# SrikarK-code/clip-dplm

Measured on AMD Instinct MI355X. Metric: seq-pairs/sec/node, contrastive training step, ESM-2-35M dual encoder, higher is better.
Workload: dtype bf16

## Files before the change

### clip_dplm_amd/_ffi.py

```python
from __future__ import annotations

import ctypes as C
import os

_HERE = os.path.dirname(os.path.abspath(__file__))
LIB_PATH = os.path.join(_HERE, "lib", "libclipk.so")

BF16, F32, U8 = 0, 1, 2
SAME_CLASS = {"mask": 0, "positive": 1}
ACT_NONE, ACT_RELU, ACT_GELU, ACT_CELU, ACT_SOFTPLUS = 0, 1, 2, 3, 4
ACT = {None: ACT_NONE, "none": ACT_NONE, "relu": ACT_RELU, "gelu": ACT_GELU, "celu": ACT_CELU, "softplus": ACT_SOFTPLUS}


class ClipkError(RuntimeError):
    pass


class GemmArgs(C.Structure):
    _fields_ = [
        ("A", C.c_void_p), ("lda", C.c_int64),
        ("B", C.c_void_p), ("ldb", C.c_int64),
        ("C", C.c_void_p), ("ldc", C.c_int64), ("c_dtype", C.c_int),
        ("M", C.c_int), ("N", C.c_int), ("K", C.c_int),
        ("bias", C.c_void_p),
        ("act", C.c_int),
        ("out_preact", C.c_void_p), ("ldp", C.c_int64),
        ("dact_aux", C.c_void_p), ("ldd", C.c_int64),
        ("dact", C.c_int),
        ("residual", C.c_void_p), ("ldr", C.c_int64), ("r_dtype", C.c_int),
        ("alpha", C.c_float),
        ("drop_p", C.c_float), ("drop_seed", C.c_uint32),
        ("rope_cos", C.c_void_p), ("rope_sin", C.c_void_p),
        ("rope_L", C.c_int), ("rope_hd", C.c_int), ("rope_cols", C.c_int), ("rope_row0", C.c_int),
        ("aux_dtype", C.c_int),
        ("rope_interleaved", C.c_int),
    ]


_vp, _i, _i64, _f, _sz = C.c_void_p, C.c_int, C.c_int64, C.c_float, C.c_size_t

SIGNATURES = {
    "clipk_version": (_i, []),
    "clipk_arch": (C.c_char_p, []),
    "clipk_status_string": (C.c_char_p, [_i]),
    "clipk_set_option": (_i, [C.c_char_p, _i]),
    "clipk_get_option": (_i, [C.c_char_p, C.POINTER(_i)]),
    "clipk_reset_options": (_i, []),
    "clipk_gemm_nt": (_i, [C.POINTER(GemmArgs), _vp]),
    "clipk_gemm_wgrad_workspace": (_sz, [_i, _i, _i]),
    "clipk_gemm_wgrad": (_i, [_vp, _i64, _vp, _i64, _vp, _i64, _vp, _i, _i, _i, _i, _i, _i, _vp, _sz, _vp]),
    "clipk_simce_workspace": (_sz, [_i, _i, _i]),
    "clipk_simce_lse": (_i, [_vp, _i, _vp, _i, _vp, _i, _i, _vp, _i, _vp, _vp, _vp, _sz, _vp]),
    "clipk_simce_grad": (_i, [_vp, _i, _vp, _i, _vp, _i, _i, _vp, _i, _vp, _vp, _f, _f, _f, _vp, _vp, _vp, _sz, _vp]),
    "clipk_simce_grad_scaled": (_i, [_vp, _i, _vp, _i, _vp, _i, _i, _vp, _i, _vp, _vp, _f, _f, _f, _vp, _vp, _vp, _vp, _sz, _vp]),
    "clipk_ce_combine": (_i, [_vp, _vp, _vp, _vp, _i, _f, _f, _f, _vp, _vp]),
    "clipk_simce_cls_workspace": (_sz, [_i, _i, _i]),
    "clipk_simce_lse_cls": (_i, [_vp, _i, _vp, _i, _vp, _i, _i, _vp, _i, _vp, _vp, _i, _f, _vp, _vp, _vp, _vp, _sz, _vp]),
    "clipk_simce_grad_cls": (_i, [_vp, _i, _vp, _i, _vp, _i, _i, _vp, _i, _vp, _vp, _vp, _vp, _vp, _vp, _i, _f, _i, _f, _f,
                                  _f, _vp, _vp, _vp, _vp, _sz, _vp]),
    "clipk_simce_hard_workspace": (_sz, [_i, _i, _i]),
    "clipk_simce_lse_hard": (_i, [_vp, _i, _vp, _i, _vp, _i, _i, _vp, _f, _i, _vp, _vp, _vp, _vp, _vp, _vp, _sz, _vp]),
    "clipk_simce_grad_hard": (_i, [_vp, _i, _vp, _i, _vp, _i, _i, _vp, _f, _i, _vp, _vp, _vp, _vp, _f, _f, _f, _vp, _vp,
                                   _vp, _vp, _sz, _vp]),
    "clipk_simce_pairs_workspace": (_sz, [_i, _i, _i]),
    "clipk_simce_lse_pairs": (_i, [_vp, _i, _i, _i, C.POINTER(_i), _i, _vp, _vp, _vp, _vp, _sz, _vp]),
# ... 99 lines not shown

def load() -> C.CDLL:
    global _lib
    if _lib is not None:
        return _lib
    if not os.path.exists(LIB_PATH):
        raise ClipkError(
            f"{LIB_PATH} not found: the HIP extension is mandatory (there is no CPU fallback). "
            "Build it with `make` or `python -c 'import __graft_entry__ as g; g.build()'`.")
    lib = C.CDLL(LIB_PATH)
    lib.clipk_version.restype = C.c_int
    got = lib.clipk_version()
    if got != ABI_VERSION:
        raise ClipkError(f"{LIB_PATH} has ABI version {got}, this binding expects {ABI_VERSION}: rebuild it (`make`)")
    for name, (res, args) in SIGNATURES.items():
        fn = getattr(lib, name)
        fn.restype = res
        fn.argtypes = args
    _lib = lib
    return lib


def check(status: int, what: str) -> None:
    if status != 0:
        msg = load().clipk_status_string(status).decode()
        raise ClipkError(f"{what} failed: {msg} (status {status})")


def ptr(t):
    return None if t is None else t.data_ptr()

# ... 5 lines not shown
```

### clip_dplm_amd/csrc/gemm_wgrad.hip

```cpp
#include "common.h"
#include <stdlib.h>

struct clipk_wgrad_v3_args {
  const unsigned short* dY; long lddy;
  const unsigned short* X; long ldx;
  float* slab; float* bslab;
  int M, N, K;
  int ntn, ntk, splits, m_per_split;
};
extern "C" void clipk_wgrad_v3_plan(int M, int N, int K, int* ntn, int* ntk, int* splits, int* mps);
extern "C" int clipk_wgrad_v3_launch(const clipk_wgrad_v3_args* a, void* stream);

namespace {

constexpr int BN = 128, BKO = 128, BMS = 64, NTHREADS = 256;
constexpr int ROWB = 256;
constexpr int TILE_BYTES = BMS * ROWB;
constexpr int LDS_BYTES = 2 * TILE_BYTES;

struct WP {
  const unsigned short* dY; long lddy;
  const unsigned short* X; long ldx;
  float* slab;
  float* bslab;
  int M, N, K;
  int ntn, ntk, splits, m_per_split;
// ... 245 lines not shown
  p.dY = (const unsigned short*)dY; p.lddy = lddy;
  p.X = (const unsigned short*)X; p.ldx = ldx;
  p.slab = (float*)workspace;
  p.bslab = dbias ? (float*)workspace + (size_t)pl.splits * N * K : nullptr;
  p.M = M; p.N = N; p.K = K;
  p.ntn = pl.ntn; p.ntk = pl.ntk; p.splits = pl.splits; p.m_per_split = pl.mps;
  hipLaunchKernelGGL(wgrad_kernel, dim3(pl.ntn * pl.ntk * pl.splits), dim3(NTHREADS), LDS_BYTES, st, p);
  int rc = clipk_check_launch();
  if (rc) return rc;
  long total4 = (long)N * K / 4;
  int blocks = (int)((total4 + 255) / 256); if (blocks > 2048) blocks = 2048; if (blocks < 1) blocks = 1;
  hipLaunchKernelGGL(wgrad_reduce_kernel, dim3(blocks), dim3(256), 0, st, (const float*)p.slab, (const float*)p.bslab,
                     pl.splits, pl.splits, N, K, dW, (long)lddw, dbias, accumulate, il_hd, il_rows);
  return clipk_check_launch();
}
```

### clip_dplm_amd/csrc/gemm_wgrad_v3.hip

```cpp
#include "common.h"
#include <stdlib.h>
#include <type_traits>

struct clipk_wgrad_v3_args {
  const unsigned short* dY; long lddy;
  const unsigned short* X; long ldx;
  float* slab;
  float* bslab;
  int M, N, K;
  int ntn, ntk, splits, m_per_split;
};

namespace {

constexpr int BN = 256, BKO = 256, BMS = 64;
constexpr int ROWB = 256;
constexpr int HALF_BYTES = BMS * ROWB;
constexpr int BUF_BYTES = 4 * HALF_BYTES;
constexpr int LDS_BYTES = 2 * BUF_BYTES;
constexpr int YH0 = 0, YH1 = HALF_BYTES, XH0 = 2 * HALF_BYTES, XH1 = 3 * HALF_BYTES;

typedef __attribute__((ext_vector_type(2))) unsigned int u32x2;

template <int OFF>
// ... 13 lines not shown
template <int KH, int NH>
__device__ __forceinline__ void quad(f32x4 (&acc)[8][4], const bf16x8 (&yf)[4][2], const bf16x8 (&xf)[2][2][2]) {
#pragma unroll
  for (int ms = 0; ms < 2; ++ms)
#pragma unroll
    for (int u = 0; u < 2; ++u)
#pragma unroll
      for (int t = 0; t < 4; ++t)
        acc[NH * 4 + t][KH * 2 + u] =
            __builtin_amdgcn_mfma_f32_16x16x32_bf16(yf[t][ms], xf[KH][u][ms], acc[NH * 4 + t][KH * 2 + u], 0, 0, 0);
}

#define CLIPK_SB() __builtin_amdgcn_sched_barrier(0)
#define CLIPK_BAR() __builtin_amdgcn_s_barrier()

template <int SCHED>
__global__ __launch_bounds__(512, 1) void wgrad_v3_kernel(const clipk_wgrad_v3_args p) {
  extern __shared__ __attribute__((aligned(16))) char smem[];
  const int tid = threadIdx.x, lane = tid & 63;
  const int wid = __builtin_amdgcn_readfirstlane(tid >> 6);
  const int wn = wid >> 2, wk = wid & 3;
  const int ntiles = p.ntn * p.ntk;
  const int bid = xcd_remap(blockIdx.x, gridDim.x);
  const int split = bid / ntiles;
  const int tile = bid - split * ntiles;
  const int tn = tile / p.ntk, tk = tile - tn * p.ntk;
  const int n0 = tn * BN, k0 = tk * BKO;
  const int M = p.M, N = p.N, K = p.K;
  const int m_beg = split * p.m_per_split;
  int m_end = m_beg + p.m_per_split; m_end = m_end < M ? m_end : M;
  const int nkt = (m_end - m_beg + BMS - 1) / BMS;
  const bool has_bias = p.bslab != nullptr;
  int bias_T = tk;

  unsigned yv[2], xv[2];
#pragma unroll
  for (int i = 0; i < 2; ++i) {
    const int row = 4 * (2 * wid + i) + (lane >> 4);
    const int slot = lane & 15;
    const int col = (((slot >> 1) ^ (row & 7)) << 4) + (slot & 1) * 8;
    yv[i] = (unsigned)(((long)row * p.lddy + (col >> 6) * 128 + (col & 63)) * 2);
    xv[i] = (unsigned)(((long)row * p.ldx + (col >> 5) * 64 + (col & 31)) * 2);
  }
  const unsigned short* y_end = p.dY + ((long)(M - 1) * p.lddy + N);
  const unsigned short* x_end = p.X + ((long)(M - 1) * p.ldx + K);
  auto stage = [&](bool is_y, int half, int T, int region) {
    const long mt = (long)m_beg + (long)T * BMS;
    const unsigned short* base = is_y ? p.dY + mt * p.lddy + (n0 + half * 64) : p.X + mt * p.ldx + (k0 + half * 32);
// ... 5 lines not shown
    for (int i = 0; i < 2; ++i)
      __builtin_amdgcn_raw_ptr_buffer_load_lds(d, (__attribute__((address_space(3))) void*)(dst + i * 1024), 16,
                                               (int)(is_y ? yv[i] : xv[i]), 0, 0, 0);
  };
  auto stage1 = [&](bool is_y, int half, int T, int region, int i) {
    const long mt = (long)m_beg + (long)T * BMS;
    const unsigned short* base = is_y ? p.dY + mt * p.lddy + (n0 + half * 64) : p.X + mt * p.ldx + (k0 + half * 32);
    const long left = ((is_y ? y_end : x_end) - base) * 2;
    const int bytes = left > 0 ? (int)(left < 0x7fffffffL ? left : 0x7fffffffL) : 0;
    const auto d = __builtin_amdgcn_make_buffer_rsrc((void*)base, 0, bytes, 0x00020000);
    char* dst = smem + (T & 1) * BUF_BYTES + region + wid * 2048 + i * 1024;
    __builtin_amdgcn_raw_ptr_buffer_load_lds(d, (__attribute__((address_space(3))) void*)dst, 16,
                                             (int)(is_y ? (i ? yv[1] : yv[0]) : (i ? xv[1] : xv[0])), 0, 0, 0);
  };

  f32x4 acc[8][4];
#pragma unroll
  for (int i = 0; i < 8; ++i)
#pragma unroll
    for (int j = 0; j < 4; ++j) acc[i][j] = f32x4{0.f, 0.f, 0.f, 0.f};
  f32x4 accb[2][2];
#pragma unroll
  for (int u = 0; u < 2; ++u) { accb[u][0] = f32x4{0.f, 0.f, 0.f, 0.f}; accb[u][1] = accb[u][0]; }
  bf16x8 ones;
#pragma unroll
  for (int j = 0; j < 8; ++j) ones[j] = (short)0x3F80;

  const int g = lane >> 4, li = lane & 15;
  const int trow = 4 * g + (li >> 2);
  const int sw = trow & 7;
  const unsigned lds0 = (unsigned)(size_t)(__attribute__((address_space(3))) char*)smem;
  unsigned ya[4], xa[2];
#pragma unroll
  for (int t = 0; t < 4; ++t) ya[t] = lds0 + trow * ROWB + (((wn * 4 + t) ^ sw) << 5) + 8 * (li & 3);
#pragma unroll
  for (int u = 0; u < 2; ++u) xa[u] = lds0 + trow * ROWB + (((wk * 2 + u) ^ sw) << 5) + 8 * (li & 3);

  if constexpr (SCHED == 1) {
// ... 219 lines not shown

    stage(true, 0, 0, YH0); stage(false, 0, 0, XH0); stage(false, 1, 0, XH1); stage(true, 1, 0, YH1);
    if (nkt > 1) {
      stage(true, 0, 1, YH0); stage(false, 0, 1, XH0); stage(false, 1, 1, XH1); stage(true, 1, 1, YH1);
      asm volatile("s_waitcnt vmcnt(8)" ::: "memory");
    } else {
      asm volatile("s_waitcnt vmcnt(0)" ::: "memory");
    }
    CLIPK_SB(); CLIPK_BAR(); CLIPK_SB();
    read_yq(I0{}, 0u); read_x(I0{}, 0u);
    for (int T = 0; T < nkt - 2; ++T) step2(std::integral_constant<int, 0>{}, T);
    if (nkt > 1) step2(std::integral_constant<int, 1>{}, nkt - 2);
    step2(std::integral_constant<int, 2>{}, nkt - 1);
  }

  float* slab = p.slab + (long)split * N * K;
#pragma unroll
  for (int i = 0; i < 8; ++i)
#pragma unroll
    for (int r = 0; r < 4; ++r) {
      const int n = n0 + wn * 128 + i * 16 + 4 * g + r;
#pragma unroll
      for (int j = 0; j < 4; ++j) {
        const int k = k0 + wk * 64 + j * 16 + li;
        if (n < N && k < K) slab[(long)n * K + k] = acc[i][j][r];
      }
    }
  if (has_bias && li == 0) {
    float* bs = p.bslab + ((long)split * p.ntk + tk) * N;
#pragma unroll
    for (int u = 0; u < 2; ++u)
#pragma unroll
      for (int r = 0; r < 4; ++r) {
        const int n = n0 + wn * 128 + u * 64 + wk * 16 + 4 * g + r;
        if (n < N) bs[n] = accb[u][0][r] + accb[u][1][r];
      }
  }
}

}

extern "C" void clipk_wgrad_v3_plan(int M, int N, int K, int* ntn, int* ntk, int* splits, int* mps) {
  *ntn = (N + BN - 1) / BN; *ntk = (K + BKO - 1) / BKO;
  const int ntiles = *ntn * *ntk;
  int s = 256 / ntiles;
  if (clipk_opt_get(OPT_WGRAD_SPLITS) > 0) s = clipk_opt_get(OPT_WGRAD_SPLITS);
  if (s < 1) s = 1;
  const int max_splits = (M + 8 * BMS - 1) / (8 * BMS);
  if (s > max_splits) s = max_splits;
  int m = (M + s - 1) / s;
  m = (m + BMS - 1) / BMS * BMS;
// ... 4 lines not shown
extern "C" int clipk_wgrad_v3_launch(const clipk_wgrad_v3_args* a, void* stream) {
  static std::atomic<uint64_t> attr_set{0};
  clipk_once_per_device(attr_set, [&] {
    (void)hipFuncSetAttribute(reinterpret_cast<const void*>(wgrad_v3_kernel<1>),
                              hipFuncAttributeMaxDynamicSharedMemorySize, LDS_BYTES);
    (void)hipFuncSetAttribute(reinterpret_cast<const void*>(wgrad_v3_kernel<2>),
                              hipFuncAttributeMaxDynamicSharedMemorySize, LDS_BYTES);
  });
  const dim3 grid(a->ntn * a->ntk * a->splits);
  if (clipk_opt_get(OPT_WGRAD_KERNEL) == 3)
    hipLaunchKernelGGL(wgrad_v3_kernel<1>, grid, dim3(512), LDS_BYTES, (hipStream_t)stream, *a);
  else
    hipLaunchKernelGGL(wgrad_v3_kernel<2>, grid, dim3(512), LDS_BYTES, (hipStream_t)stream, *a);
  return clipk_check_launch();
}
```

### clip_dplm_amd/encoders.py

```python
from __future__ import annotations

import math
from typing import List, Optional

import os

import torch
import torch.nn as nn

from . import functional as KF
from . import ops


def _rope_tables(L: int, hd: int, device, theta: float = 10000.0):
    inv = 1.0 / (theta ** (torch.arange(0, hd, 2, dtype=torch.float32) / hd))
    fr = torch.arange(L, dtype=torch.float32)[:, None] * inv[None, :]
    return fr.cos().contiguous().to(device), fr.sin().contiguous().to(device)


WGRAD_SIDE_STREAM = False
_SIDE = {}


PREROTATE_QK = os.environ.get("CLIPK_PREROTATE", "1") != "0"
ROPE_IN_QKV_EPILOGUE = os.environ.get("CLIPK_ROPE_EPILOGUE", "1") != "0"
DIRECT_PARAM_GRADS = True
ROPE_INTERLEAVED = os.environ.get("CLIPK_ROPE_INTERLEAVED", "1") != "0"


def _direct_ok(t):
    g = t.grad if (t is not None and t.is_leaf) else None
    return g is not None and g.dtype == torch.float32 and g.is_contiguous() and g.device == t.device


def _fused_views(parts):
    p0 = parts[0]
    if not all(q.is_leaf and q.requires_grad and q.grad is not None and q.is_contiguous() and q.grad.is_contiguous()
               and q.dtype == torch.float32 and q.grad.dtype == torch.float32 for q in parts):
        return None
    d_ptr, g_ptr = p0.data_ptr(), p0.grad.data_ptr()
    for q in parts:
# ... 14 lines not shown

def _ln_bwd(dy, x, w, b, mean, rstd, pool=None, **kw):
    if pool is not None:
        wrow, B, L = pool
        if DIRECT_PARAM_GRADS and _direct_ok(w) and _direct_ok(b):
            dx, dxb, _, _ = ops.layernorm_meanpool_bwd(dy, wrow, x, w, mean, rstd, B, L, dgamma=w.grad, dbeta=b.grad,
                                                       accumulate=True, **kw)
            return dx, dxb, None, None
        return ops.layernorm_meanpool_bwd(dy, wrow, x, w, mean, rstd, B, L, **kw)
    if DIRECT_PARAM_GRADS and _direct_ok(w) and _direct_ok(b):
        dx, dxb, _, _ = ops.layernorm_bwd(dy, x, w, None, mean, rstd, dgamma=w.grad, dbeta=b.grad, accumulate=True, **kw)
        return dx, dxb, None, None
    return ops.layernorm_bwd(dy, x, w, None, mean, rstd, **kw)


def _wgrad(dy, x, lin=None, il=(0, 0)):
    if DIRECT_PARAM_GRADS and lin is not None and lin.gw is not None and lin.gb is not None:
        direct, kw = True, dict(dw=lin.gw, dbias=lin.gb, accumulate=True)
    else:
        direct = DIRECT_PARAM_GRADS and lin is not None and _direct_ok(lin.w) and _direct_ok(lin.b)
        kw = dict(dw=lin.w.grad, dbias=lin.b.grad, accumulate=True) if direct else dict(want_bias=True)
    if il[1]:
        kw["il"] = il
    if not (WGRAD_SIDE_STREAM and dy.is_cuda):
        r = ops.gemm_wgrad(dy, x, **kw)
        return (None, None) if direct else r
    cur = torch.cuda.current_stream()
    side = _SIDE.get(cur.cuda_stream)
    if side is None:
        side = _SIDE[cur.cuda_stream] = torch.cuda.Stream()
    side.wait_event(cur.record_event())
# ... 119 lines not shown
    else:
        g, u = ops.gemm_nt(h2, p["fc1"].wb, bias=p["fc1"].b, act="gelu"), None
    y = ops.gemm_nt(g, p["fc2"].wb, bias=p["fc2"].b, residual=x2, out_dtype=torch.float32)
    return y, (x, h1, m1, r1, qkv, ctx, lse, x2, h2, m2, r2, g, u)


ESM_BF16_GRAD_STREAM = os.environ.get("CLIPK_ESM_F32_GRAD_STREAM", "0") != "1"


def _esm_layer_bwd(dy, dyb, p, saved, attn, need_dx_bf16, need_dx_f32=True):
    x, h1, m1, r1, qkv, ctx, lse, x2, h2, m2, r2, g, u = saved
    if dyb is None:
        dyb = ops.to_bf16(dy)
    lowp = dy is None
    gr = {}
    du = ops.gemm_nt(dyb, p["fc2"].wtb, dact_aux=u, dact="gelu")
    gr["fc2_w"], gr["fc2_b"] = _wgrad(dyb, g, p["fc2"])
    dh2 = ops.gemm_nt(du, p["fc1"].wtb)
    gr["fc1_w"], gr["fc1_b"] = _wgrad(du, h2, p["fc1"])
    dx2, dx2b, gr["ln2_w"], gr["ln2_b"] = _ln_bwd(dh2, x2, p["ln2_w"], p["ln2_b"], m2, r2, dx_add=dyb if lowp else dy,
                                                  want_f32=not lowp, want_bf16=True)
    dctx = ops.gemm_nt(dx2b, p["out"].wtb)
    gr["out_w"], gr["out_b"] = _wgrad(dx2b, ctx, p["out"])
    dqkv = attn.bwd(qkv, ctx, dctx, lse)
    dh1 = ops.gemm_nt(dqkv, p["qkv"].wtb)
    gr["qkv_w"], gr["qkv_b"] = _wgrad(dqkv, h1, p["qkv"], il=p["qkv"].il)
    want32 = need_dx_f32 or not lowp
    dx, dxb, gr["ln1_w"], gr["ln1_b"] = _ln_bwd(dh1, x, p["ln1_w"], p["ln1_b"], m1, r1, dx_add=dx2b if lowp else dx2,
                                                want_f32=want32, want_bf16=need_dx_bf16 or lowp)
    return dx, dxb, gr


_ESM_KEYS = ["ln1_w", "ln1_b", "qkv_w", "qkv_b", "out_w", "out_b", "ln2_w", "ln2_b", "fc1_w", "fc1_b", "fc2_w", "fc2_b"]


class EsmStackFn(torch.autograd.Function):

    @staticmethod
    def forward(ctx, module, ids, mask_u8, row_scale, seq, pool, *flat):
        nl = module.num_layers
        table, fin_w, fin_b = flat[0], flat[1], flat[2]
# ... 266 lines not shown
        _, yb, m2, r2 = ops.layernorm_fwd(s2, p["n2_w"], p["n2_b"], eps, want_f32=False, want_bf16=True)
        y = yb
    else:
        y, yb, m2, r2 = ops.layernorm_fwd(s2, p["n2_w"], p["n2_b"], eps, want_f32=True, want_bf16=True)
    return y, yb, (xb, qkv, ctx, lse, s1, x1b, m1, r1, g, u, s2, m2, r2)


def _post_layer_bwd(dy, p, saved, meta, dr=None, need_dx=True):
    attn, act, eps, res16 = meta
    da, d1, df, d2 = (None,) * 4 if dr is None else tuple((dr[0], sd) for sd in dr[1:])
    xb, qkv, ctx, lse, s1, x1b, m1, r1, g, u, s2, m2, r2 = saved
    gr = {}
    lowp = res16 and dr is None
    ds2, ds2b, gr["n2_w"], gr["n2_b"] = _ln_bwd(dy, s2, p["n2_w"], p["n2_b"], m2, r2, want_f32=not lowp, want_bf16=True,
                                                dropout_bf16=d2)
    du = ops.gemm_nt(ds2b, p["fc2"].wtb, dact_aux=u, dact=act, dropout=df)
    gr["fc2_w"], gr["fc2_b"] = _wgrad(ds2b, g, p["fc2"])
    if lowp:
        dx1 = ops.gemm_nt(du, p["fc1"].wtb, residual=ds2b)
    else:
        dx1 = ops.gemm_nt(du, p["fc1"].wtb, residual=ds2, out_dtype=torch.float32)
    gr["fc1_w"], gr["fc1_b"] = _wgrad(du, x1b, p["fc1"])
    ds1, ds1b, gr["n1_w"], gr["n1_b"] = _ln_bwd(dx1, s1, p["n1_w"], p["n1_b"], m1, r1, want_f32=not lowp, want_bf16=True,
                                                dropout_bf16=d1)
    dctx = ops.gemm_nt(ds1b, p["out"].wtb)
    gr["out_w"], gr["out_b"] = _wgrad(ds1b, ctx, p["out"])
    dqkv = attn.bwd(qkv, ctx, dctx, lse, dropout=da)
    if not need_dx:
        dx = None
    elif lowp:
        dx = ops.gemm_nt(dqkv, p["in"].wtb, residual=ds1b)
    else:
        dx = ops.gemm_nt(dqkv, p["in"].wtb, residual=ds1, out_dtype=torch.float32)
    gr["in_w"], gr["in_b"] = _wgrad(dqkv, xb, p["in"])
    return dx, gr


_POST_KEYS = ["in_w", "in_b", "out_w", "out_b", "n1_w", "n1_b", "fc1_w", "fc1_b", "fc2_w", "fc2_b", "n2_w", "n2_b"]


class PostLNStackFn(torch.autograd.Function):

    @staticmethod
    def forward(ctx, module, x, mask_u8, B, L, seq, drop, pool, *flat):
        nl = module.num_layers
        E, H = module.embed_dim, module.nhead
        D = module.head_dim_padded
        meta = (_Attn(B, L, H, D, mask_u8, seq, float(E // H) ** -0.5), module.activation, module.eps,
                module.residual_dtype == "bf16" and POSTLN_BF16_RESIDUAL)
# ... 228 lines not shown
```

### clip_dplm_amd/ops.py

```python
from __future__ import annotations

import ctypes as C
from typing import NamedTuple, Optional

import torch

from . import _ffi
from ._ffi import ACT, BF16, F32, U8, GemmArgs, check, ptr

_WS: dict = {}


class KernelTimer:

    def __init__(self, only=None):
        self.records = {}
        self.only = None if only is None else set(only)

    def add(self, name, s, e, work, nbytes=0.0, sub=None):
        self.records.setdefault(name, []).append((s, e, work, nbytes, sub))

    def summary_by_sub(self, name):
        groups = {}
        for r in self.records.get(name, []):
# ... 185 lines not shown
    if dw is None:
        dw = torch.empty((N, K), dtype=torch.float32, device=dy.device)
        accumulate = False
    if want_bias and dbias is None:
        dbias = torch.empty((N,), dtype=torch.float32, device=dy.device)
    lib = _lib()
    nbytes = lib.clipk_gemm_wgrad_workspace(M, N, K)
    ws = workspace(nbytes, dy.device, "wgrad")
    check(_timed("gemm_wgrad", 2.0 * M * N * K,
                 lambda: lib.clipk_gemm_wgrad(dy.data_ptr(), dy.stride(0), x.data_ptr(), x.stride(0), dw.data_ptr(),
                                              dw.stride(0), ptr(dbias), M, N, K, int(accumulate), int(il[0]), int(il[1]),
                                              ws.data_ptr(), ws.numel(), _stream())), "clipk_gemm_wgrad")
    return dw, dbias


_SIMCE_KINDS = {"plain": ("clipk_simce_workspace", "simce"),
                "cls": ("clipk_simce_cls_workspace", "simce (class-aware)"),
                "hard": ("clipk_simce_hard_workspace", "simce (hard-negative)")}


def _simce(entry, kind, x, y, scale, cache, args, outs):
    Mx, P = x.shape
    Ny = y.shape[0]
    Nc = 0 if cache is None else cache.shape[0]
    dev = x.device
    res = [new(*shape, dtype=torch.float32, device=dev) for new, shape in outs]
    lib = _lib()
    ws_entry, what = _SIMCE_KINDS[kind]
    nbytes = getattr(lib, ws_entry)(Mx, Ny + Nc, P)
    if nbytes == 0:
# ... 1320 lines not shown
```

### include/clipk.h

```cpp
#ifndef CLIPK_H
#define CLIPK_H

#include <stddef.h>
#include <stdint.h>

#ifdef __cplusplus
extern "C" {
#endif

typedef enum clipk_status {
  CLIPK_OK = 0,
  CLIPK_ERR_BAD_ARG = -1,
  CLIPK_ERR_UNSUPPORTED = -2,
  CLIPK_ERR_LAUNCH = -3
} clipk_status;

typedef enum clipk_dtype { CLIPK_BF16 = 0, CLIPK_F32 = 1, CLIPK_U8 = 2 } clipk_dtype;
typedef enum clipk_act { CLIPK_ACT_NONE = 0, CLIPK_ACT_RELU = 1, CLIPK_ACT_GELU = 2, CLIPK_ACT_CELU = 3,
                         CLIPK_ACT_SOFTPLUS = 4 } clipk_act;

int clipk_version(void);
const char* clipk_arch(void);
const char* clipk_status_string(int status);

// ... 14 lines not shown
  const void* residual; int64_t ldr; int r_dtype;
  float alpha;
  float drop_p; uint32_t drop_seed;
  const float* rope_cos; const float* rope_sin; int rope_L, rope_hd, rope_cols, rope_row0;
  int aux_dtype;
  int rope_interleaved;
} clipk_gemm_args;
int clipk_gemm_nt(const clipk_gemm_args* args, void* stream);

size_t clipk_gemm_wgrad_workspace(int M, int N, int K);
int clipk_gemm_wgrad(const void* dY, int64_t lddy, const void* X, int64_t ldx,
                     float* dW, int64_t lddw, float* dbias,
                     int M, int N, int K, int accumulate, int il_hd, int il_rows,
                     void* workspace, size_t workspace_bytes, void* stream);

size_t clipk_simce_workspace(int Mx, int Nkeys, int P);
int clipk_simce_lse(const float* X, int Mx, const float* Y, int Ny, const float* Yc, int Nc,
                    int P, const float* scale ,
                    int label_offset, float* lse , float* pos ,
                    void* workspace, size_t workspace_bytes, void* stream);

int clipk_simce_grad(const float* X, int Mx, const float* Y, int Ny, const float* Yc, int Nc,
                     int P, const float* scale, int label_offset,
                     const float* lse_x, const float* lse_y, float w_row, float w_col, float inv_bg,
                     float* dX , float* dscale_partial ,
                     void* workspace, size_t workspace_bytes, void* stream);
int clipk_simce_grad_scaled(const float* X, int Mx, const float* Y, int Ny, const float* Yc, int Nc,
                            int P, const float* scale, int label_offset,
                            const float* lse_x, const float* lse_y, float w_row, float w_col, float inv_bg,
                            const float* upstream, float* dX , float* dscale_partial ,
// ... 262 lines not shown
```

Measured before the change: 6420.

## Group per-layer weight-gradient GEMMs into one stream-K style grouped launch

The four weight-gradient GEMMs of each transformer layer's backward (fc2, fc1, out, qkv/in) are now deferred and issued as a single grouped kernel. Output tiles from all problems are split along M into segments that are spread over a fixed number of workgroups, followed by one reduction kernel that sums the partial slabs into dW and dbias. This aims to cut per-GEMM launch and tail-imbalance overhead and keep more CUs busy on small ESM-2-35M wgrads. In exchange it adds slab traffic and a reduction pass, and the wgrads are delayed until the end of the layer, so they no longer interleave with the data-gradient GEMMs.

```diff
diff --git a/clip_dplm_amd/_ffi.py b/clip_dplm_amd/_ffi.py
--- a/clip_dplm_amd/_ffi.py
+++ b/clip_dplm_amd/_ffi.py
@@ -37,7 +37,19 @@
     ]
 
 
+class WgradProblem(C.Structure):
+    _fields_ = [
+        ("dY", C.c_void_p), ("lddy", C.c_int64),
+        ("X", C.c_void_p), ("ldx", C.c_int64),
+        ("dW", C.c_void_p), ("lddw", C.c_int64),
+        ("dbias", C.c_void_p),
+        ("M", C.c_int), ("N", C.c_int), ("K", C.c_int),
+        ("il_hd", C.c_int), ("il_rows", C.c_int),
+    ]
+
+
 _vp, _i, _i64, _f, _sz = C.c_void_p, C.c_int, C.c_int64, C.c_float, C.c_size_t
+_ip = C.POINTER(C.c_int)
 
 SIGNATURES = {
     "clipk_version": (_i, []),
@@ -49,6 +61,11 @@
     "clipk_gemm_nt": (_i, [C.POINTER(GemmArgs), _vp]),
     "clipk_gemm_wgrad_workspace": (_sz, [_i, _i, _i]),
     "clipk_gemm_wgrad": (_i, [_vp, _i64, _vp, _i64, _vp, _i64, _vp, _i, _i, _i, _i, _i, _i, _vp, _sz, _vp]),
+    "clipk_gemm_wgrad_grouped_workspace": (_sz, [C.POINTER(WgradProblem), _i, _i]),
+    "clipk_gemm_wgrad_grouped": (_i, [C.POINTER(WgradProblem), _i, _i, _i, _vp, _sz, _vp]),
+    "clipk_wgrad_group_layout": (_i, [_i, _i, _i, _ip, _ip, _ip]),
+    "clipk_wgrad_group_segments": (_i, [_i, _i, _i, _i, _i, _i, _vp, _i, _i, _vp]),
+    "clipk_wgrad_group_tile_partials": (_i, [_i, _i, _i, _i, _i, _ip, _i]),
     "clipk_simce_workspace": (_sz, [_i, _i, _i]),
     "clipk_simce_lse": (_i, [_vp, _i, _vp, _i, _vp, _i, _i, _vp, _i, _vp, _vp, _vp, _sz, _vp]),
     "clipk_simce_grad": (_i, [_vp, _i, _vp, _i, _vp, _i, _i, _vp, _i, _vp, _vp, _f, _f, _f, _vp, _vp, _vp, _sz, _vp]),
@@ -178,7 +195,10 @@
     if got != ABI_VERSION:
         raise ClipkError(f"{LIB_PATH} has ABI version {got}, this binding expects {ABI_VERSION}: rebuild it (`make`)")
     for name, (res, args) in SIGNATURES.items():
-        fn = getattr(lib, name)
+        try:
+            fn = getattr(lib, name)
+        except AttributeError:
+            raise ClipkError(f"{LIB_PATH} lacks {name}, which this binding declares: rebuild it (`make`)") from None
         fn.restype = res
         fn.argtypes = args
     _lib = lib
diff --git a/clip_dplm_amd/csrc/gemm_wgrad.hip b/clip_dplm_amd/csrc/gemm_wgrad.hip
--- a/clip_dplm_amd/csrc/gemm_wgrad.hip
+++ b/clip_dplm_amd/csrc/gemm_wgrad.hip
@@ -10,6 +10,8 @@
 };
 extern "C" void clipk_wgrad_v3_plan(int M, int N, int K, int* ntn, int* ntk, int* splits, int* mps);
 extern "C" int clipk_wgrad_v3_launch(const clipk_wgrad_v3_args* a, void* stream);
+#include "wgrad_group_plan.h"
+extern "C" int clipk_wgrad_v3_group_launch(const wgrad_group_args* a, void* stream);
 
 namespace {
 
@@ -285,3 +287,95 @@
                      pl.splits, pl.splits, N, K, dW, (long)lddw, dbias, accumulate, il_hd, il_rows);
   return clipk_check_launch();
 }
+
+namespace {
+constexpr int GROUP_WGS = 256;
+
+int group_plan(const clipk_wgrad_problem* pr, int np, int group_wgs, wgrad_group_args* a) {
+  if (!pr || np < 1 || np > CLIPK_WGRAD_GROUP_MAX || group_wgs < 0) return CLIPK_ERR_BAD_ARG;
+  const int M = pr[0].M;
+  int T = 0;
+  for (int i = 0; i < np; ++i) {
+    const clipk_wgrad_problem& q = pr[i];
+    if (!q.dY || !q.X || !q.dW || q.M != M || q.M <= 0 || q.N <= 0 || q.K <= 0) return CLIPK_ERR_BAD_ARG;
+    if (q.il_rows < 0 || q.il_rows > q.N || (q.il_rows > 0 && (q.il_hd < 2 || (q.il_hd & 1) || q.il_rows % q.il_hd)))
+      return CLIPK_ERR_BAD_ARG;
+    if ((q.N & 7) || (q.K & 7) || (q.lddy & 7) || (q.ldx & 7) || (q.lddw & 3)) return CLIPK_ERR_BAD_ARG;
+    if (!aligned16(q.dY) || !aligned16(q.X) || !aligned16(q.dW)) return CLIPK_ERR_BAD_ARG;
+    if (!use_v3(q.M, q.N, q.K)) return CLIPK_ERR_BAD_ARG;
+    wgrad_group_prob& d = a->pr[i];
+    d.dY = (const unsigned short*)q.dY; d.lddy = (long)q.lddy;
+    d.X = (const unsigned short*)q.X; d.ldx = (long)q.ldx;
+    d.dW = q.dW; d.lddw = (long)q.lddw; d.dbias = q.dbias;
+    d.N = q.N; d.K = q.K; d.ntn = (q.N + 255) / 256; d.ntk = (q.K + 255) / 256;
+    d.tile0 = T;
+    d.il_hd = q.il_rows ? q.il_hd : 2; d.il_rows = q.il_rows;
+    T += d.ntn * d.ntk;
+  }
+  for (int i = np; i < CLIPK_WGRAD_GROUP_MAX; ++i) a->pr[i] = wgrad_group_prob{};
+  const int G = group_wgs ? group_wgs : GROUP_WGS;
+  if (T > G && !group_wgs) return CLIPK_ERR_BAD_ARG;
+  a->L = wgrad_group_choose(T, (M + BMS - 1) / BMS, G);
+  if (a->L.W < 1 || a->L.W > CLIPK_WGRAD_GROUP_MAX_W) return CLIPK_ERR_BAD_ARG;
+  a->np = np; a->M = M;
+  return CLIPK_OK;
+}
+size_t group_bytes(const wgrad_group_layout& L) { return (size_t)wgrad_group_slots(L) * (256 * 256 + 256) * sizeof(float); }
+}
+
+extern "C" size_t clipk_gemm_wgrad_grouped_workspace(const clipk_wgrad_problem* problems, int nproblems, int group_wgs) {
+  wgrad_group_args a;
+  if (group_plan(problems, nproblems, group_wgs, &a) != CLIPK_OK) return 0;
+  return group_bytes(a.L);
+}
+
+extern "C" int clipk_gemm_wgrad_grouped(const clipk_wgrad_problem* problems, int nproblems, int accumulate, int group_wgs,
+                                        void* workspace, size_t workspace_bytes, void* stream) {
+  wgrad_group_args a;
+  const int rc = group_plan(problems, nproblems, group_wgs, &a);
+  if (rc) return rc;
+  if (!workspace || !aligned16(workspace) || workspace_bytes < group_bytes(a.L)) return CLIPK_ERR_BAD_ARG;
+  a.accumulate = accumulate;
+  a.slab = (float*)workspace;
+  a.bslab = a.slab + (size_t)wgrad_group_slots(a.L) * (256 * 256);
+  return clipk_wgrad_v3_group_launch(&a, stream);
+}
+
+namespace {
+__host__ __device__ inline int group_walk(const wgrad_group_layout& L, int band, int j, int* out, int max_seg) {
+  int pos = wgrad_group_bound(L, j), n = 0;
+  const int hi = wgrad_group_bound(L, j + 1);
+  while (pos < hi) {
+    wgrad_group_segment sg;
+    pos = wgrad_group_segment_at(L, band, j, pos, hi, &sg);
+    if (n < max_seg) { out[4 * n] = sg.tile; out[4 * n + 1] = sg.t0; out[4 * n + 2] = sg.n; out[4 * n + 3] = sg.slot; }
+    ++n;
+  }
+  return n;
+}
+__global__ void group_walk_kernel(wgrad_group_layout L, int band, int j, int* out, int max_seg) {
+  out[4 * max_seg] = group_walk(L, band, j, out, max_seg);
+}
+}
+
+extern "C" int clipk_wgrad_group_layout(int tiles, int steps_per_tile, int group_wgs, int* D, int* W, int* slots) {
+  if (tiles < 1 || steps_per_tile < 1 || group_wgs < 1 || !D || !W || !slots) return CLIPK_ERR_BAD_ARG;
+  const wgrad_group_layout L = wgrad_group_choose(tiles, steps_per_tile, group_wgs);
+  *D = L.D; *W = L.W; *slots = wgrad_group_slots(L);
+  return CLIPK_OK;
+}
+extern "C" int clipk_wgrad_group_segments(int tiles, int steps_per_tile, int D, int W, int band, int j, int* out,
+                                          int max_seg, int device, void* stream) {
+  if (tiles < 1 || steps_per_tile < 1 || D < 1 || W < 1 || tiles % D || band < 0 || band >= tiles / D || j < 0 || j >= W ||
+      !out || max_seg < 0)
+    return CLIPK_ERR_BAD_ARG;
+  const wgrad_group_layout L{tiles, steps_per_tile, D, W};
+  if (!device) return group_walk(L, band, j, out, max_seg);
+  hipLaunchKernelGGL(group_walk_kernel, dim3(1), dim3(1), 0, (hipStream_t)stream, L, band, j, out, max_seg);
+  return clipk_check_launch();
+}
+extern "C" int clipk_wgrad_group_tile_partials(int tiles, int steps_per_tile, int D, int W, int tile, int* slots, int max_n) {
+  if (tiles < 1 || steps_per_tile < 1 || D < 1 || W < 1 || tiles % D || tile < 0 || tile >= tiles || !slots) return CLIPK_ERR_BAD_ARG;
+  const wgrad_group_layout L{tiles, steps_per_tile, D, W};
+  return wgrad_group_tile_partials(L, tile, slots, max_n);
+}
diff --git a/clip_dplm_amd/csrc/gemm_wgrad_v3.hip b/clip_dplm_amd/csrc/gemm_wgrad_v3.hip
--- a/clip_dplm_amd/csrc/gemm_wgrad_v3.hip
+++ b/clip_dplm_amd/csrc/gemm_wgrad_v3.hip
@@ -1,6 +1,7 @@
 #include "common.h"
 #include <stdlib.h>
 #include <type_traits>
+#include "wgrad_group_plan.h"
 
 struct clipk_wgrad_v3_args {
   const unsigned short* dY; long lddy;
@@ -51,24 +52,24 @@
 #define CLIPK_SB() __builtin_amdgcn_sched_barrier(0)
 #define CLIPK_BAR() __builtin_amdgcn_s_barrier()
 
+struct wgrad_v3_tile {
+  const unsigned short* dY; long lddy;
+  const unsigned short* X; long ldx;
+  int M, N, K;
+  int n0, k0;
+  int ntk;
+  bool has_bias;
+};
+
 template <int SCHED>
-__global__ __launch_bounds__(512, 1) void wgrad_v3_kernel(const clipk_wgrad_v3_args p) {
-  extern __shared__ __attribute__((aligned(16))) char smem[];
-  const int tid = threadIdx.x, lane = tid & 63;
+__device__ __forceinline__ void wgrad_v3_mainloop(const int tid, char* smem, const wgrad_v3_tile& p, const int m_beg,
+                                                  const int nkt, int bias_T, f32x4 (&acc)[8][4], f32x4 (&accb)[2][2]) {
+  const int lane = tid & 63;
   const int wid = __builtin_amdgcn_readfirstlane(tid >> 6);
   const int wn = wid >> 2, wk = wid & 3;
-  const int ntiles = p.ntn * p.ntk;
-  const int bid = xcd_remap(blockIdx.x, gridDim.x);
-  const int split = bid / ntiles;
-  const int tile = bid - split * ntiles;
-  const int tn = tile / p.ntk, tk = tile - tn * p.ntk;
-  const int n0 = tn * BN, k0 = tk * BKO;
+  const int n0 = p.n0, k0 = p.k0;
   const int M = p.M, N = p.N, K = p.K;
-  const int m_beg = split * p.m_per_split;
-  int m_end = m_beg + p.m_per_split; m_end = m_end < M ? m_end : M;
-  const int nkt = (m_end - m_beg + BMS - 1) / BMS;
-  const bool has_bias = p.bslab != nullptr;
-  int bias_T = tk;
+  const bool has_bias = p.has_bias;
 
   unsigned yv[2], xv[2];
 #pragma unroll
@@ -104,14 +105,6 @@
                                              (int)(is_y ? (i ? yv[1] : yv[0]) : (i ? xv[1] : xv[0])), 0, 0, 0);
   };
 
-  f32x4 acc[8][4];
-#pragma unroll
-  for (int i = 0; i < 8; ++i)
-#pragma unroll
-    for (int j = 0; j < 4; ++j) acc[i][j] = f32x4{0.f, 0.f, 0.f, 0.f};
-  f32x4 accb[2][2];
-#pragma unroll
-  for (int u = 0; u < 2; ++u) { accb[u][0] = f32x4{0.f, 0.f, 0.f, 0.f}; accb[u][1] = accb[u][0]; }
   bf16x8 ones;
 #pragma unroll
   for (int j = 0; j < 8; ++j) ones[j] = (short)0x3F80;
@@ -361,27 +354,150 @@
     step2(std::integral_constant<int, 2>{}, nkt - 1);
   }
 
-  float* slab = p.slab + (long)split * N * K;
+}
+
+#define CLIPK_WGRAD_ZERO_ACC()                                                                      \
+  _Pragma("unroll") for (int i = 0; i < 8; ++i)                                                     \
+    _Pragma("unroll") for (int j = 0; j < 4; ++j) acc[i][j] = f32x4{0.f, 0.f, 0.f, 0.f};            \
+  _Pragma("unroll") for (int u = 0; u < 2; ++u) { accb[u][0] = f32x4{0.f, 0.f, 0.f, 0.f}; accb[u][1] = accb[u][0]; }
+
+__device__ __forceinline__ void wgrad_v3_store(const int tid, const f32x4 (&acc)[8][4], const f32x4 (&accb)[2][2],
+                                               float* dst, long ld, float* bdst, int n0, int k0, int N, int K) {
+  const int lane = tid & 63;
+  const int wid = __builtin_amdgcn_readfirstlane(tid >> 6);
+  const int wn = wid >> 2, wk = wid & 3;
+  const int g = lane >> 4, li = lane & 15;
 #pragma unroll
   for (int i = 0; i < 8; ++i)
 #pragma unroll
     for (int r = 0; r < 4; ++r) {
-      const int n = n0 + wn * 128 + i * 16 + 4 * g + r;
+      const int nl = wn * 128 + i * 16 + 4 * g + r;
 #pragma unroll
       for (int j = 0; j < 4; ++j) {
-        const int k = k0 + wk * 64 + j * 16 + li;
-        if (n < N && k < K) slab[(long)n * K + k] = acc[i][j][r];
+        const int kl = wk * 64 + j * 16 + li;
+        if (n0 + nl < N && k0 + kl < K) dst[(long)nl * ld + kl] = acc[i][j][r];
       }
     }
-  if (has_bias && li == 0) {
-    float* bs = p.bslab + ((long)split * p.ntk + tk) * N;
+  if (bdst && li == 0) {
 #pragma unroll
     for (int u = 0; u < 2; ++u)
 #pragma unroll
       for (int r = 0; r < 4; ++r) {
-        const int n = n0 + wn * 128 + u * 64 + wk * 16 + 4 * g + r;
-        if (n < N) bs[n] = accb[u][0][r] + accb[u][1][r];
-      }
+        const int nl = wn * 128 + u * 64 + wk * 16 + 4 * g + r;
+        if (n0 + nl < N) bdst[nl] = accb[u][0][r] + accb[u][1][r];
+      }
+  }
+}
+
+template <int SCHED>
+__global__ __launch_bounds__(512, 1) void wgrad_v3_kernel(const clipk_wgrad_v3_args p) {
+  extern __shared__ __attribute__((aligned(16))) char smem[];
+  const int ntiles = p.ntn * p.ntk;
+  const int bid = xcd_remap(blockIdx.x, gridDim.x);
+  const int split = bid / ntiles;
+  const int tile = bid - split * ntiles;
+  const int tn = tile / p.ntk, tk = tile - tn * p.ntk;
+  const int n0 = tn * BN, k0 = tk * BKO;
+  const int M = p.M, N = p.N, K = p.K;
+  const int m_beg = split * p.m_per_split;
+  int m_end = m_beg + p.m_per_split; m_end = m_end < M ? m_end : M;
+  const int nkt = (m_end - m_beg + BMS - 1) / BMS;
+  const wgrad_v3_tile t{p.dY, p.lddy, p.X, p.ldx, M, N, K, n0, k0, p.ntk, p.bslab != nullptr};
+  f32x4 acc[8][4];
+  f32x4 accb[2][2];
+  CLIPK_WGRAD_ZERO_ACC();
+  wgrad_v3_mainloop<SCHED>(threadIdx.x, smem, t, m_beg, nkt, tk, acc, accb);
+  wgrad_v3_store(threadIdx.x, acc, accb, p.slab + (long)split * N * K + ((long)n0 * K + k0), K,
+                 t.has_bias ? p.bslab + ((long)split * p.ntk + tk) * N + n0 : nullptr, n0, k0, N, K);
+}
+
+__global__ __launch_bounds__(512, 1) void wgrad_grouped_kernel(const wgrad_group_args a) {
+  extern __shared__ __attribute__((aligned(16))) char smem[];
+  const wgrad_group_layout L = a.L;
+  const int nb = wgrad_group_bands(L);
+  const int lid = xcd_remap(blockIdx.x, gridDim.x);
+  const int j = lid / nb, i = lid - j * nb;
+  const int wave = __builtin_amdgcn_readfirstlane(threadIdx.x >> 6);
+  int pos = wgrad_group_bound(L, j);
+  const int hi = wgrad_group_bound(L, j + 1);
+  bool again = false;
+  while (pos < hi) {
+    wgrad_group_segment sg;
+    pos = wgrad_group_segment_at(L, i, j, pos, hi, &sg);
+    int pi = 0;
+    while (pi + 1 < a.np && sg.tile >= a.pr[pi + 1].tile0) ++pi;
+    const wgrad_group_prob& q = a.pr[pi];
+    const int tile = sg.tile - q.tile0;
+    const int tn = tile / q.ntk, tk = tile - tn * q.ntk;
+    const wgrad_v3_tile t{q.dY, q.lddy, q.X, q.ldx, a.M, q.N, q.K, tn * BN, tk * BKO, q.ntk, q.dbias != nullptr};
+    int bias_T = tk - sg.t0 % q.ntk;
+    bias_T += bias_T < 0 ? q.ntk : 0;
+    if (again) __syncthreads();
+    again = true;
+    int tid = wave * WAVE + (int)__builtin_amdgcn_mbcnt_hi(~0u, __builtin_amdgcn_mbcnt_lo(~0u, 0u));
+    asm volatile("" : "+v"(tid));
+    f32x4 acc[8][4], accb[2][2];
+    CLIPK_WGRAD_ZERO_ACC();
+    wgrad_v3_mainloop<2>(tid, smem, t, sg.t0 * BMS, sg.n, bias_T, acc, accb);
+    wgrad_v3_store(tid, acc, accb, a.slab + (long)sg.slot * (BN * BKO), BKO,
+                   t.has_bias ? a.bslab + (long)sg.slot * BN : nullptr, t.n0, t.k0, t.N, t.K);
+  }
+}
+
+__global__ __launch_bounds__(256) void wgrad_grouped_reduce_kernel(const wgrad_group_args a) {
+  __shared__ int sl[CLIPK_WGRAD_GROUP_MAX_W];
+  __shared__ int cnt;
+  const wgrad_group_layout L = a.L;
+  const int gt = blockIdx.x >> 6, chunk = blockIdx.x & 63;
+  const int tid = threadIdx.x;
+  int pi = 0;
+  while (pi + 1 < a.np && gt >= a.pr[pi + 1].tile0) ++pi;
+  const wgrad_group_prob& q = a.pr[pi];
+  const int tile = gt - q.tile0;
+  const int tn = tile / q.ntk, tk = tile - tn * q.ntk;
+  const int n0 = tn * BN, k0 = tk * BKO;
+  auto list_partials = [&](int t) {
+    if (tid == 0) cnt = wgrad_group_tile_partials(L, t, sl, CLIPK_WGRAD_GROUP_MAX_W);
+    __syncthreads();
+  };
+  list_partials(gt);
+  const int np = cnt;
+  const int c4 = tid & 63;
+  const int row = chunk * 4 + (tid >> 6);
+  const int n = n0 + row, k = k0 + 4 * c4;
+  if (n < q.N && k < q.K) {
+    const f32x4* src = reinterpret_cast<const f32x4*>(a.slab + (long)row * BKO) + c4;
+    constexpr long TS = BN * BKO / 4;
+    f32x4 s4 = f32x4{0.f, 0.f, 0.f, 0.f};
+    int s = 0;
+    for (; s + 4 <= np; s += 4) {
+      const f32x4 v0 = src[sl[s] * TS], v1 = src[sl[s + 1] * TS], v2 = src[sl[s + 2] * TS], v3 = src[sl[s + 3] * TS];
+      s4 += (v0 + v1) + (v2 + v3);
+    }
+    for (; s < np; ++s) s4 += src[sl[s] * TS];
+    f32x4* o = reinterpret_cast<f32x4*>(q.dW + (long)il_src(n, q.il_hd, q.il_rows) * q.lddw + k);
+    *o = a.accumulate ? (*o + s4) : s4;
+  }
+  if (chunk == 0 && tk == 0 && q.dbias) {
+    float b = 0.f;
+    for (int t2 = 0; t2 < q.ntk; ++t2) {
+      __syncthreads();
+      list_partials(gt + t2);
+      const int nbp = cnt;
+      const float* src = a.bslab + tid;
+      int s = 0;
+      for (; s + 4 <= nbp; s += 4) {
+        const float v0 = src[(long)sl[s] * BN], v1 = src[(long)sl[s + 1] * BN], v2 = src[(long)sl[s + 2] * BN],
+                    v3 = src[(long)sl[s + 3] * BN];
+        b += (v0 + v1) + (v2 + v3);
+      }
+      for (; s < nbp; ++s) b += src[(long)sl[s] * BN];
+    }
+    const int n = n0 + tid;
+    if (n < q.N) {
+      const int o = il_src(n, q.il_hd, q.il_rows);
+      q.dbias[o] = a.accumulate ? q.dbias[o] + b : b;
+    }
   }
 }
 
@@ -416,3 +532,17 @@
     hipLaunchKernelGGL(wgrad_v3_kernel<2>, grid, dim3(512), LDS_BYTES, (hipStream_t)stream, *a);
   return clipk_check_launch();
 }
+
+extern "C" int clipk_wgrad_v3_group_launch(const wgrad_group_args* a, void* stream) {
+  static std::atomic<uint64_t> attr_set{0};
+  clipk_once_per_device(attr_set, [&] {
+    (void)hipFuncSetAttribute(reinterpret_cast<const void*>(wgrad_grouped_kernel),
+                              hipFuncAttributeMaxDynamicSharedMemorySize, LDS_BYTES);
+  });
+  const int nwg = wgrad_group_bands(a->L) * a->L.W;
+  hipLaunchKernelGGL(wgrad_grouped_kernel, dim3(nwg), dim3(512), LDS_BYTES, (hipStream_t)stream, *a);
+  int rc = clipk_check_launch();
+  if (rc) return rc;
+  hipLaunchKernelGGL(wgrad_grouped_reduce_kernel, dim3(a->L.T * 64), dim3(256), 0, (hipStream_t)stream, *a);
+  return clipk_check_launch();
+}
diff --git a/clip_dplm_amd/csrc/wgrad_group_plan.h b/clip_dplm_amd/csrc/wgrad_group_plan.h
--- /dev/null
+++ b/clip_dplm_amd/csrc/wgrad_group_plan.h
@@ -0,0 +1,95 @@
+#pragma once
+
+#if defined(__HIPCC__)
+#define CLIPK_WG_HD __host__ __device__
+#else
+#define CLIPK_WG_HD
+#endif
+
+constexpr int CLIPK_WGRAD_GROUP_MAX = 8;
+constexpr int CLIPK_WGRAD_GROUP_MAX_W = 1024;
+constexpr int CLIPK_WGRAD_GROUP_SNAP = 8;
+
+struct wgrad_group_layout {
+  int T;
+  int spt;
+  int D;
+  int W;
+};
+CLIPK_WG_HD inline int wgrad_group_bands(const wgrad_group_layout& L) { return L.T / L.D; }
+CLIPK_WG_HD inline int wgrad_group_slots(const wgrad_group_layout& L) { return wgrad_group_bands(L) * (L.W + L.D - 1); }
+
+CLIPK_WG_HD inline int wgrad_group_bound(const wgrad_group_layout& L, int j) {
+  const long long Sb = (long long)L.D * L.spt;
+  if (j <= 0) return 0;
+  if (j >= L.W) return (int)Sb;
+  const int pos = (int)((long long)j * Sb / L.W);
+  const int r = pos % L.spt;
+  if (r < CLIPK_WGRAD_GROUP_SNAP) return pos - r;
+  if (L.spt - r < CLIPK_WGRAD_GROUP_SNAP) return pos + (L.spt - r);
+  return pos;
+}
+
+struct wgrad_group_segment {
+  int tile;
+  int t0;
+  int n;
+  int slot;
+};
+CLIPK_WG_HD inline int wgrad_group_segment_at(const wgrad_group_layout& L, int i, int j, int pos, int hi,
+                                              wgrad_group_segment* s) {
+  const int r = pos / L.spt;
+  int end = (r + 1) * L.spt;
+  end = end < hi ? end : hi;
+  s->tile = r * wgrad_group_bands(L) + i;
+  s->t0 = pos - r * L.spt;
+  s->n = end - pos;
+  s->slot = i * (L.W + L.D - 1) + j + r;
+  return end;
+}
+CLIPK_WG_HD inline bool wgrad_group_touches(const wgrad_group_layout& L, int j, int r) {
+  int lo = wgrad_group_bound(L, j), hi = wgrad_group_bound(L, j + 1);
+  const int ts = r * L.spt, te = ts + L.spt;
+  lo = lo > ts ? lo : ts;
+  hi = hi < te ? hi : te;
+  return lo < hi;
+}
+CLIPK_WG_HD inline int wgrad_group_tile_partials(const wgrad_group_layout& L, int tile, int* slots, int max_n) {
+  const int nb = wgrad_group_bands(L), i = tile % nb, r = tile / nb;
+  int n = 0;
+  for (int j = 0; j < L.W; ++j)
+    if (wgrad_group_touches(L, j, r)) {
+      if (n < max_n) slots[n] = i * (L.W + L.D - 1) + j + r;
+      ++n;
+    }
+  return n;
+}
+
+inline wgrad_group_layout wgrad_group_choose(int T, int spt, int G) {
+  wgrad_group_layout L{T, spt, T, G};
+  if (G < T) return L;
+  L.D = 1; L.W = G / T;
+  for (int d = 2; d <= 4; ++d) {
+    if (T % d) continue;
+    const int w = (int)((long long)G * d / T);
+    if ((long long)w * L.D > (long long)L.W * d) { L.D = d; L.W = w; }
+  }
+  return L;
+}
+
+struct wgrad_group_prob {
+  const unsigned short* dY; long lddy;
+  const unsigned short* X; long ldx;
+  float* dW; long lddw;
+  float* dbias;
+  int N, K, ntn, ntk;
+  int tile0;
+  int il_hd, il_rows;
+};
+struct wgrad_group_args {
+  wgrad_group_prob pr[CLIPK_WGRAD_GROUP_MAX];
+  wgrad_group_layout L;
+  int np, M, accumulate;
+  float* slab;
+  float* bslab;
+};
diff --git a/clip_dplm_amd/encoders.py b/clip_dplm_amd/encoders.py
--- a/clip_dplm_amd/encoders.py
+++ b/clip_dplm_amd/encoders.py
@@ -25,6 +25,7 @@
 PREROTATE_QK = os.environ.get("CLIPK_PREROTATE", "1") != "0"
 ROPE_IN_QKV_EPILOGUE = os.environ.get("CLIPK_ROPE_EPILOGUE", "1") != "0"
 DIRECT_PARAM_GRADS = True
+WGRAD_GROUPED = True
 ROPE_INTERLEAVED = os.environ.get("CLIPK_ROPE_INTERLEAVED", "1") != "0"
 
 
@@ -69,7 +70,33 @@
     return ops.layernorm_bwd(dy, x, w, None, mean, rstd, **kw)
 
 
-def _wgrad(dy, x, lin=None, il=(0, 0)):
+def _direct_bufs(lin):
+    if not DIRECT_PARAM_GRADS or lin is None:
+        return None
+    if lin.gw is not None and lin.gb is not None:
+        return lin.gw, lin.gb
+    return (lin.w.grad, lin.b.grad) if _direct_ok(lin.w) and _direct_ok(lin.b) else None
+
+
+def _wgrad_group(dy, *lins):
+    if not (WGRAD_GROUPED and not WGRAD_SIDE_STREAM and dy.is_cuda):
+        return None
+    return [] if all(_direct_bufs(lin) is not None for lin in lins) else None
+
+
+def _wgrad_flush(group):
+    if not group:
+        return
+    probs = [(dy, x) + _direct_bufs(lin) + (il,) for dy, x, lin, il in group]
+    if not ops.gemm_wgrad_grouped(probs, accumulate=True):
+        for dy, x, lin, il in group:
+            _wgrad(dy, x, lin, il)
+
+
+def _wgrad(dy, x, lin=None, il=(0, 0), group=None):
+    if group is not None:
+        group.append((dy, x, lin, il))
+        return None, None
     if DIRECT_PARAM_GRADS and lin is not None and lin.gw is not None and lin.gb is not None:
         direct, kw = True, dict(dw=lin.gw, dbias=lin.gb, accumulate=True)
     else:
@@ -219,17 +246,19 @@
         dyb = ops.to_bf16(dy)
     lowp = dy is None
     gr = {}
+    grp = _wgrad_group(dyb, p["fc2"], p["fc1"], p["out"], p["qkv"])
     du = ops.gemm_nt(dyb, p["fc2"].wtb, dact_aux=u, dact="gelu")
-    gr["fc2_w"], gr["fc2_b"] = _wgrad(dyb, g, p["fc2"])
+    gr["fc2_w"], gr["fc2_b"] = _wgrad(dyb, g, p["fc2"], group=grp)
     dh2 = ops.gemm_nt(du, p["fc1"].wtb)
-    gr["fc1_w"], gr["fc1_b"] = _wgrad(du, h2, p["fc1"])
+    gr["fc1_w"], gr["fc1_b"] = _wgrad(du, h2, p["fc1"], group=grp)
     dx2, dx2b, gr["ln2_w"], gr["ln2_b"] = _ln_bwd(dh2, x2, p["ln2_w"], p["ln2_b"], m2, r2, dx_add=dyb if lowp else dy,
                                                   want_f32=not lowp, want_bf16=True)
     dctx = ops.gemm_nt(dx2b, p["out"].wtb)
-    gr["out_w"], gr["out_b"] = _wgrad(dx2b, ctx, p["out"])
+    gr["out_w"], gr["out_b"] = _wgrad(dx2b, ctx, p["out"], group=grp)
     dqkv = attn.bwd(qkv, ctx, dctx, lse)
     dh1 = ops.gemm_nt(dqkv, p["qkv"].wtb)
-    gr["qkv_w"], gr["qkv_b"] = _wgrad(dqkv, h1, p["qkv"], il=p["qkv"].il)
+    gr["qkv_w"], gr["qkv_b"] = _wgrad(dqkv, h1, p["qkv"], il=p["qkv"].il, group=grp)
+    _wgrad_flush(grp)
     want32 = need_dx_f32 or not lowp
     dx, dxb, gr["ln1_w"], gr["ln1_b"] = _ln_bwd(dh1, x, p["ln1_w"], p["ln1_b"], m1, r1, dx_add=dx2b if lowp else dx2,
                                                 want_f32=want32, want_bf16=need_dx_bf16 or lowp)
@@ -526,17 +555,18 @@
     lowp = res16 and dr is None
     ds2, ds2b, gr["n2_w"], gr["n2_b"] = _ln_bwd(dy, s2, p["n2_w"], p["n2_b"], m2, r2, want_f32=not lowp, want_bf16=True,
                                                 dropout_bf16=d2)
+    grp = _wgrad_group(ds2b, p["fc2"], p["fc1"], p["out"], p["in"])
     du = ops.gemm_nt(ds2b, p["fc2"].wtb, dact_aux=u, dact=act, dropout=df)
-    gr["fc2_w"], gr["fc2_b"] = _wgrad(ds2b, g, p["fc2"])
+    gr["fc2_w"], gr["fc2_b"] = _wgrad(ds2b, g, p["fc2"], group=grp)
     if lowp:
         dx1 = ops.gemm_nt(du, p["fc1"].wtb, residual=ds2b)
     else:
         dx1 = ops.gemm_nt(du, p["fc1"].wtb, residual=ds2, out_dtype=torch.float32)
-    gr["fc1_w"], gr["fc1_b"] = _wgrad(du, x1b, p["fc1"])
+    gr["fc1_w"], gr["fc1_b"] = _wgrad(du, x1b, p["fc1"], group=grp)
     ds1, ds1b, gr["n1_w"], gr["n1_b"] = _ln_bwd(dx1, s1, p["n1_w"], p["n1_b"], m1, r1, want_f32=not lowp, want_bf16=True,
                                                 dropout_bf16=d1)
     dctx = ops.gemm_nt(ds1b, p["out"].wtb)
-    gr["out_w"], gr["out_b"] = _wgrad(ds1b, ctx, p["out"])
+    gr["out_w"], gr["out_b"] = _wgrad(ds1b, ctx, p["out"], group=grp)
     dqkv = attn.bwd(qkv, ctx, dctx, lse, dropout=da)
     if not need_dx:
         dx = None
@@ -544,7 +574,8 @@
         dx = ops.gemm_nt(dqkv, p["in"].wtb, residual=ds1b)
     else:
         dx = ops.gemm_nt(dqkv, p["in"].wtb, residual=ds1, out_dtype=torch.float32)
-    gr["in_w"], gr["in_b"] = _wgrad(dqkv, xb, p["in"])
+    gr["in_w"], gr["in_b"] = _wgrad(dqkv, xb, p["in"], group=grp)
+    _wgrad_flush(grp)
     return dx, gr
 
 
diff --git a/clip_dplm_amd/ops.py b/clip_dplm_amd/ops.py
--- a/clip_dplm_amd/ops.py
+++ b/clip_dplm_amd/ops.py
@@ -223,6 +223,30 @@
     return dw, dbias
 
 
+def gemm_wgrad_grouped(problems, accumulate: bool = True, group_wgs: int = 0) -> bool:
+    lib = _lib()
+    arr = (_ffi.WgradProblem * len(problems))()
+    flops = 0.0
+    for q, (dy, x, dw, dbias, il) in zip(arr, problems):
+        _need_cuda(dy, x, dw, dbias)
+        assert dy.dtype == torch.bfloat16 and x.dtype == torch.bfloat16 and dw.dtype == torch.float32
+        assert dy.stride(1) == 1 and x.stride(1) == 1 and dw.stride(1) == 1 and dy.shape[0] == x.shape[0]
+        assert dw.shape == (dy.shape[1], x.shape[1]) and (dbias is None or (dbias.dtype == torch.float32 and dbias.is_contiguous()))
+        q.dY, q.lddy, q.X, q.ldx = dy.data_ptr(), dy.stride(0), x.data_ptr(), x.stride(0)
+        q.dW, q.lddw, q.dbias = dw.data_ptr(), dw.stride(0), ptr(dbias)
+        q.M, q.N, q.K = dy.shape[0], dy.shape[1], x.shape[1]
+        q.il_hd, q.il_rows = int(il[0]), int(il[1])
+        flops += 2.0 * q.M * q.N * q.K
+    nbytes = lib.clipk_gemm_wgrad_grouped_workspace(arr, len(problems), int(group_wgs))
+    if nbytes == 0:
+        return False
+    ws = workspace(nbytes, problems[0][0].device, "wgrad_grouped")
+    check(_timed("gemm_wgrad", flops,
+                 lambda: lib.clipk_gemm_wgrad_grouped(arr, len(problems), int(accumulate), int(group_wgs), ws.data_ptr(),
+                                                      ws.numel(), _stream())), "clipk_gemm_wgrad_grouped")
+    return True
+
+
 _SIMCE_KINDS = {"plain": ("clipk_simce_workspace", "simce"),
                 "cls": ("clipk_simce_cls_workspace", "simce (class-aware)"),
                 "hard": ("clipk_simce_hard_workspace", "simce (hard-negative)")}
diff --git a/include/clipk.h b/include/clipk.h
--- a/include/clipk.h
+++ b/include/clipk.h
@@ -52,6 +52,22 @@
                      int M, int N, int K, int accumulate, int il_hd, int il_rows,
                      void* workspace, size_t workspace_bytes, void* stream);
 
+typedef struct clipk_wgrad_problem {
+  const void* dY; int64_t lddy;
+  const void* X; int64_t ldx;
+  float* dW; int64_t lddw;
+  float* dbias;
+  int M, N, K;
+  int il_hd, il_rows;
+} clipk_wgrad_problem;
+size_t clipk_gemm_wgrad_grouped_workspace(const clipk_wgrad_problem* problems, int nproblems, int group_wgs);
+int clipk_gemm_wgrad_grouped(const clipk_wgrad_problem* problems, int nproblems, int accumulate, int group_wgs,
+                             void* workspace, size_t workspace_bytes, void* stream);
+int clipk_wgrad_group_layout(int tiles, int steps_per_tile, int group_wgs, int* D, int* W, int* slots);
+int clipk_wgrad_group_segments(int tiles, int steps_per_tile, int D, int W, int band, int j, int* out, int max_seg,
+                               int device, void* stream);
+int clipk_wgrad_group_tile_partials(int tiles, int steps_per_tile, int D, int W, int tile, int* slots, int max_n);
+
 size_t clipk_simce_workspace(int Mx, int Nkeys, int P);
 int clipk_simce_lse(const float* X, int Mx, const float* Y, int Ny, const float* Yc, int Nc,
                     int P, const float* scale ,
```

After: 6468, median of 6. No clear change (+0.7%).
